# nilsbore/gp_compressor

Measured on AMD Instinct MI355X. Metric: patches/sec (compress+predict), higher is better.
Workload: dtype f64; 1 GPU; C2 room scan: 8192 patches x 256 pts per GPU, RBF + Gaussian noise, dense Cholesky fit + predictive mean on the 20x20 grid (m=400); patches_per_gpu=8192, points_per_patch=256, grid_points=400, parallelism=1 GPU, kernel=dense_mfma_w1

## Files before the change

### gp_compressor_amd/capi.py

```python
import ctypes as C
import os
import weakref

import numpy as np

HERE = os.path.dirname(os.path.abspath(__file__))
LIB_PATH = os.environ.get("GPC_LIB_PATH", os.path.join(HERE, "libgpc_hip.so"))

GPC_OK, GPC_EINVAL, GPC_ENOMEM, GPC_ENODEV, GPC_EHIP, GPC_ERANGE = 0, -22, -12, -19, -5, -34
CELL_UNOBSERVED, CELL_OCCUPIED, CELL_FREE = 0, 1, 2
STATUS_OK, STATUS_NOT_SPD, STATUS_NAN, STATUS_SIGMA_CLAMPED, STATUS_OVERFLOW, STATUS_NOT_CONVERGED = 0, 1, 2, 3, 4, 5
MAX_POINTS, MAX_BV = 1024, 256

c_dp = C.POINTER(C.c_double)
c_ip = C.POINTER(C.c_int32)


class Params(C.Structure):
    _fields_ = [("sigmaf_sq", C.c_double), ("l_sq", C.c_double), ("noise", C.c_double), ("eps_tol", C.c_double),
                ("capacity", C.c_int32), ("noise_model", C.c_int32), ("ref_double_noise", C.c_int32),
                ("ref_field_delete_bug", C.c_int32), ("want_variance", C.c_int32), ("reserved", C.c_int32)]


class IrlsParams(C.Structure):
# ... 143 lines not shown
    "gpc_registration_get_cloud": (C.c_int, [_vp, _vp]),
    "gpc_registration_cloud_dev": (C.c_int, [_vp, C.POINTER(_vp), C.POINTER(C.c_int)]),
    "gpc_registration_get_assignment": (C.c_int, [_vp, _vp, _vp]),
    "gpc_partition_patches": (C.c_int, [_i, _vp, _i, _i, _vp]),
    "gpc_comm_unique_id": (C.c_int, [_vp]),
    "gpc_comm_create": (C.c_int, [_vp, _i, _i, _vp, C.POINTER(_vp)]),
    "gpc_comm_create_all": (C.c_int, [_i, C.POINTER(_vp), C.POINTER(_vp)]),
    "gpc_comm_adopt": (C.c_int, [_vp, _vp, _i, _i, C.POINTER(_vp)]),
    "gpc_comm_destroy": (None, [_vp]),
    "gpc_comm_world": (C.c_int, [_vp]),
    "gpc_comm_rank": (C.c_int, [_vp]),
    "gpc_comm_library": (C.c_char_p, []),
    "gpc_comm_set_partition": (C.c_int, [_vp, _i, _vp]),
    "gpc_group_start": (C.c_int, []),
    "gpc_group_end": (C.c_int, []),
    "gpc_allgather_fstar_dev": (C.c_int, [_vp, _i, _vp, _vp, _vp]),
    "gpc_unpermute_fstar_dev": (C.c_int, [_vp, _i, _vp, _vp]),
    "gpc_test_exp_host": (None, [_vp, _vp, _i]),
    "gpc_test_exp_small_host": (None, [_vp, _vp, _i]),
    "gpc_test_quantize_host": (C.c_int, [_vp, _i, _i, _vp, _vp, _vp]),
    "gpc_test_rate_allocate_host": (C.c_int, [_i, _i, _vp, _vp, _vp, _vp, _d, _vp, _i, C.c_int64, _i, _vp, _vp, _vp, _vp]),
    "gpc_test_par_memcpy": (None, [_vp, _vp, C.c_size_t]),
    "gpc_test_dense_route": (C.c_int, [_i] * 11 + [_vp, _i, _vp]),
}

_lib = None


def load():
    global _lib
    if _lib is not None:
        return _lib
    try:
        import torch
    except ImportError:
        pass
    if not os.path.exists(LIB_PATH):
        raise GpcError(GPC_ENODEV, f"{LIB_PATH} not built: run `python -c 'import __graft_entry__ as g; g.build()'` "
                                   "(hipcc --offload-arch=gfx950); there is no CPU fallback")
    lib = C.CDLL(LIB_PATH)
    for name, (res, args) in PROTOTYPES.items():
        fn = getattr(lib, name)
        fn.restype = res
        fn.argtypes = args
    _lib = lib
    return lib
# ... 129 lines not shown
    def free_host_array(self, a):
        p = getattr(self, "_pinned", {}).pop(a.ctypes.data, None)
        if p is not None:
            self._check(self.lib.gpc_host_free(self.h, p))

    def rate_allocate(self, kmax, d0, d, need, w=None, w_all=1.0, unit=None, unit_all=24, refine=True, count=None):
        a = _rate_args(kmax, d0, d, w, unit, count)
        R, ld = a[2].shape
        k = np.zeros(R, dtype=np.int32)
        tg = None if count is None else np.zeros(R, dtype=np.int32)
        res = np.zeros(1, dtype=RATE_RESULT_DTYPE)
        self._check(self.lib.gpc_rate_allocate(self.h, R, ld, _ptr(a[0]), _ptr(a[1]), _ptr(a[2]), _ptr(a[3]), float(w_all), _ptr(a[4]),
                                               int(unit_all), int(need), int(bool(refine)), _ptr(a[5]), _ptr(k), _ptr(tg), _ptr(res)))
        return (k, rate_result(res)) if count is None else (k, tg, rate_result(res))

    def rate_allocate_dev(self, R, ld, kmax, d0, d, need, w=None, w_all=1.0, unit=None, unit_all=24, refine=True, count=None, k=None,
                          target=None, result=None):
        self._check(self.lib.gpc_rate_allocate_dev(self.h, int(R), int(ld), _ptr(kmax), _ptr(d0), _ptr(d), _ptr(w), float(w_all),
                                                   _ptr(unit), int(unit_all), int(need), int(bool(refine)), _ptr(count), _ptr(k),
                                                   _ptr(target), _ptr(result)))

    def last_dense_kernel(self):
        return self.lib.gpc_last_dense_kernel(self.h).decode()

    def dense_fit_predict(self, params, off, x0, x1, y, xs0, xs1, want_alpha=False):
        off = np.ascontiguousarray(off, dtype=np.int32)
        y = np.ascontiguousarray(np.atleast_2d(y), dtype=np.float64)
        x0 = np.ascontiguousarray(x0, dtype=np.float64)
        x1 = np.ascontiguousarray(x1, dtype=np.float64)
        xs0 = np.ascontiguousarray(xs0, dtype=np.float64)
        xs1 = np.ascontiguousarray(xs1, dtype=np.float64)
        P, ny, m = off.shape[0] - 1, y.shape[0], xs0.shape[0]
        f = np.full((P, ny, m), np.nan)
        v = np.full((P, m), np.nan) if params.want_variance else None
        st = np.full(P, -1, dtype=np.int32)
        al = np.full_like(y, np.nan) if want_alpha else None
        self._check(self.lib.gpc_dense_fit_predict(self.h, C.byref(params), P, _ptr(off), _ptr(x0), _ptr(x1), _ptr(y), ny,
                                                   m, _ptr(xs0), _ptr(xs1), _ptr(f), _ptr(v), _ptr(al), _ptr(st)))
        return (f, v, st, al) if want_alpha else (f, v, st)

    def dense_fit_predict_grid(self, params, off, x0, x1, y, res, sz, want_alpha=False):
        off = np.ascontiguousarray(off, dtype=np.int32)
        y = np.ascontiguousarray(np.atleast_2d(y), dtype=np.float64)
        x0 = np.ascontiguousarray(x0, dtype=np.float64)
        x1 = np.ascontiguousarray(x1, dtype=np.float64)
        P, ny, m = off.shape[0] - 1, y.shape[0], sz * sz
# ... 1080 lines not shown
    tg = None if count is None else np.zeros(R, dtype=np.int32)
    res = np.zeros(1, dtype=RATE_RESULT_DTYPE)
    rc = load().gpc_test_rate_allocate_host(R, ld, _ptr(a[0]), _ptr(a[1]), _ptr(a[2]), _ptr(a[3]), float(w_all), _ptr(a[4]), int(unit_all),
                                            int(need), int(bool(refine)), _ptr(a[5]), _ptr(k), _ptr(tg), _ptr(res))
    if rc != GPC_OK:
        raise GpcError(rc, "gpc_test_rate_allocate_host")
    return (k, rate_result(res)) if count is None else (k, tg, rate_result(res))


test_rate_allocate_host.__test__ = False


ROUTE_KINDS = {-1: "no route", 0: "nothing", 1: "one-wave", 2: "register", 3: "tiled", 4: "generic", 5: "split"}
ROUTE_SHAPE = ("w1_npad", "w1_slots", "nt", "export_factor", "waves", "npad", "per_cu", "nt17", "need_big")


def dense_route(P, n_max, n_total=None, ny=1, m=16, variance=False, pointwise=False, alpha_out=False, num_cus=256, irls=False,
                w1_refused=False):
    name = C.create_string_buffer(96)
    shape = np.zeros(len(ROUTE_SHAPE), dtype=np.int32)
    kind = load().gpc_test_dense_route(P, n_max, P * n_max if n_total is None else n_total, ny, m, int(variance), int(pointwise),
                                       int(alpha_out), num_cus, int(irls), int(w1_refused), name, len(name), _ptr(shape))
    return ROUTE_KINDS[kind], name.value.decode(), dict(zip(ROUTE_SHAPE, shape.tolist()))
```

### gp_compressor_amd/csrc/dense_api.hip

```cpp
#include "dense_internal.h"

int dense_check(gpc_ctx* ctx, const gpc_params* prm, int P, const void* off, int n_max, int n_total,
                const void* x0, const void* x1, const void* y, int ny, int m, const void* f_star)
{
    if (!ctx || ctx->dead.load()) return GPC_EINVAL;
    if (!prm) return gpc_fail(ctx, GPC_EINVAL, "params is NULL");
    if (P < 0 || m < 0 || n_total < 0 || n_max < 0) return gpc_fail(ctx, GPC_EINVAL, "negative size");
    if (ny != 1 && ny != 3) return gpc_fail(ctx, GPC_EINVAL, "ny must be 1 (depth) or 3 (RGB), got %d", ny);
    if (P > 0 && !off) return gpc_fail(ctx, GPC_EINVAL, "off is NULL");
    if (n_total > 0 && (!x0 || !x1 || !y)) return gpc_fail(ctx, GPC_EINVAL, "x0/x1/y is NULL");
    if (P > 0 && m > 0 && !f_star) return gpc_fail(ctx, GPC_EINVAL, "f_star is NULL");
    if (n_max > GPC_MAX_POINTS) return gpc_fail(ctx, GPC_ERANGE, "n_max %d > GPC_MAX_POINTS %d", n_max, GPC_MAX_POINTS);
    if (!(prm->l_sq > 0.0) || !(prm->sigmaf_sq >= 0.0) || !(prm->noise >= 0.0))
        return gpc_fail(ctx, GPC_EINVAL, "kernel/noise parameters out of range");
    return GPC_OK;
}

DenseArgs dense_args(const gpc_params* prm, int P, const int32_t* off, int n_max, int n_total, const double* x0, const double* x1,
                     const double* y, int ny, int m, double* f_star, double* alpha_out, int32_t* status)
{
    DenseArgs a{};
    a.prm = *prm;
    a.P = P; a.n_max = n_max; a.n_total = n_total; a.ny = ny; a.m = m;
    a.off = off; a.x0 = x0; a.x1 = x1; a.y = y;
// ... 75 lines not shown
    if (nt17 && (rc = run_class(1, c1, on_in)) != GPC_OK) return bail(rc);
    if ((rc = run_class(0, c0, site)) != GPC_OK) return bail(rc);
    GPC_HIP(ctx, hipEventRecord(ctx->ev[1][GPC_EV_CLASS_FORK], ctx->s_in));
    GPC_HIP(ctx, hipEventRecord(ctx->ev[2][GPC_EV_CLASS_FORK], ctx->s_out));
    GPC_HIP(ctx, hipStreamWaitEvent(main_s, ctx->ev[1][GPC_EV_CLASS_FORK], 0));
    GPC_HIP(ctx, hipStreamWaitEvent(main_s, ctx->ev[2][GPC_EV_CLASS_FORK], 0));
    return rc;
}

int dense_dispatch(gpc_ctx* ctx, DenseArgs& a, const DenseSite& site, unsigned* seen_gen)
{
    const DenseSwitches sw = dense_switches_read();
    const DenseFacts facts = dense_facts(ctx, a);
    DenseRoute route = dense_route(facts, sw);
    if (route.kind == DENSE_NOTHING) return GPC_OK;
    if (a.n_max < 1) a.n_max = 1;
    if (seen_gen)
        if (int rco = gpc_pipe_chunk_order(ctx, site.stream, seen_gen)) return rco;
    GPC_HIP(ctx, hipSetDevice(ctx->device));
    if (!a.prm.want_variance) a.v_star = nullptr;
    if (int rcp = gpc_debug_poison_lds(ctx, site)) return rcp;
    int grid = 0, rc = GPC_OK;
    if (route.kind == DENSE_ONE_WAVE) {
        for (int cap_w1 = site.w1_cap;;) {
            rc = gpc_ws_reserve(ctx, site, al256(dense_w1_ws_bytes(facts, route, &grid, cap_w1)));
            if (rc != GPC_ENOMEM) break;
            cap_w1 = grid / 2;
            if (cap_w1 < 4 * ctx->num_cus) break;
        }
        if (rc == GPC_ENOMEM) {
            route = dense_route(facts, sw, true);
            if (route.kind == DENSE_NO_ROUTE) return rc;
            (void)hipGetLastError();
        } else if (rc != GPC_OK) {
            return rc;
        }
    }
    switch (route.kind) {
        case DENSE_ONE_WAVE:
            rc = dense_w1_launch(ctx, site, a, route, grid);
            break;
        case DENSE_REGISTER:
            rc = dense_mfma_launch(ctx, site, a, route);
            break;
        case DENSE_TILED:
            if ((rc = gpc_ws_reserve(ctx, site, al256(dense_big_ws_bytes(ctx, a, route, &grid)))) == GPC_OK)
                rc = dense_big_launch(ctx, site, a, route, grid);
            break;
        case DENSE_SPLIT:
// ... 65 lines not shown
    if (ctx && (sz < 0 || sz > 1024)) return gpc_fail(ctx, GPC_EINVAL, "sz out of range");
    int rc = dense_check(ctx, params, P, off, n_max, n_total, x0, x1, y, ny, sz * sz, f_star);
    if (rc != GPC_OK) return rc;
    DenseArgs a = dense_args(params, P, off, n_max, n_total, x0, x1, y, ny, sz * sz, f_star, alpha_out, status);
    a.prm.want_variance = 0;
    a.grid_res = res; a.grid_sz = sz;
    std::lock_guard<std::mutex> lk(ctx->mu);
    return dense_dispatch(ctx, a, dense_site_of(ctx));
}

int gpc_test_dense_route(int P, int n_max, int n_total, int ny, int m, int variance, int pointwise, int alpha_out, int num_cus, int irls,
                         int w1_refused, char* name, int name_cap, int32_t* shape)
{
    const DenseFacts f{P, n_max, n_total, ny, m, variance != 0, pointwise != 0, alpha_out != 0, num_cus, irls != 0};
    const DenseRoute r = dense_route(f, dense_switches_read(), w1_refused != 0);
    if (name && name_cap > 0) snprintf(name, (size_t)name_cap, "%s", r.name);
    if (shape) {
        const int32_t v[GPC_TEST_ROUTE_SHAPE] = {r.w1_npad, r.w1_slots, r.nt, r.export_factor, r.waves, r.npad, r.per_cu, r.nt17, r.need_big};
        memcpy(shape, v, sizeof(v));
    }
    return (int)r.kind;
}

}
```

### gp_compressor_amd/csrc/dense_host.hip

```cpp
#include <algorithm>
#include <condition_variable>
#include <cstdlib>
#include <thread>
#include <vector>

#include "dense_internal.h"

namespace {
class CopyPool {
public:
    static CopyPool& get()
    {
        static CopyPool p;
        return p;
    }
    void copy(void* dst, const void* src, size_t bytes)
    {
        if (bytes < (1u << 20) || th_.empty()) { std::memcpy(dst, src, bytes); return; }
        std::lock_guard<std::mutex> call(call_mu_);
        std::unique_lock<std::mutex> lk(m_);
        dst_ = (char*)dst; src_ = (const char*)src; bytes_ = bytes;
        remaining_ = (int)th_.size();
        ++gen_;
        lk.unlock();
// ... 103 lines not shown
    struct PipeFlag {
        gpc_ctx* c;
        bool on;
        ~PipeFlag()
        {
            if (!on) return;
            std::lock_guard<std::mutex> lk(c->mu);
            c->pipe_active = false;
        }
    } pipe{ctx, false};
    {
        std::lock_guard<std::mutex> lk(ctx->mu);
        DenseFacts chunk{(P + 7) / 8, n_max, n_total, ny, m, want_v, !grid && xs0, false, ctx->num_cus, false};
        bool all_w1 = C == 4 && P >= 8192 && n_max > 160 && !alpha_out && !sw.host_one_stream && ctx->own_stream != nullptr;
        for (int c = 0; c < 8 && all_w1; ++c) {
            const int p0 = (int)((long long)P * c / 8), p1 = (int)((long long)P * (c + 1) / 8);
            DenseFacts fc = chunk;
            fc.P = p1 - p0;
            fc.n_max = 1;
            for (int i = p0; i < p1; ++i) fc.n_max = std::max(fc.n_max, off[i + 1] - off[i]);
            all_w1 = dense_route(fc, sw).kind == DENSE_ONE_WAVE;
        }
        if (all_w1) {
            half = (dense_w1_ws_bytes(chunk, dense_route(chunk, sw), nullptr) + 255) & ~(size_t)255;
            if (gpc_ws_reserve(ctx, 2 * half) == GPC_OK) {
                two = true;
                C = 8;
                pipe.on = ctx->pipe_active = true;
                seen_gen[0] = seen_gen[1] = ctx->foreign_gen;
            } else {
                (void)hipGetLastError();
            }
        }
    }
    auto al256 = [](size_t v) { return (v + 255) & ~(size_t)255; };
    const size_t b_off = al256(sizeof(int32_t) * (size_t)(P + C)), b_x = al256(8 * N), b_y = al256(8 * N * ny), b_xs = al256(8 * (size_t)m),
                 b_f = al256(8 * (size_t)P * ny * m), b_v = want_v ? al256(8 * (size_t)P * m) : 0, b_al = alpha_out ? al256(8 * N * ny) : 0,
                 b_st = al256(sizeof(int32_t) * (size_t)P);
    if ((rc = grow(ctx, &ctx->io, &ctx->io_bytes, b_off + 2 * b_x + b_y + 2 * b_xs + b_f + b_v + b_al + b_st, false))) return rc;
    char* d = static_cast<char*>(ctx->io);
    int32_t* d_off = (int32_t*)d; d += b_off;
    double* d_x0 = (double*)d; d += b_x;
    double* d_x1 = (double*)d; d += b_x;
    double* d_y = (double*)d; d += b_y;
    double* d_xs0 = (double*)d; d += b_xs;
    double* d_xs1 = (double*)d; d += b_xs;
    double* d_f = (double*)d; d += b_f;
// ... 137 lines not shown
```

### gp_compressor_amd/csrc/dense_internal.h

```cpp
#pragma once

#include "gpc_internal.h"
#include "dense_route.h"

struct DenseArgs {
    gpc_params prm;
    int P, n_max, n_total, ny, m;
    const int32_t* off;
    const double *x0, *x1, *y;
    const double *xs0, *xs1;
    double grid_res;
    int grid_sz;
    double *f_star, *v_star, *alpha_out;
    int32_t* status;
    const int32_t* sel;
    const int32_t* sel_count;
    int sel_base;
    double* log_ev;
};

struct DenseSite {
    hipStream_t stream;
    size_t ws_off, ws_len;
    int w1_cap = 0;
// ... 62 lines not shown
struct GaussRows {
    double *f;
    double *v;
    double *alpha;
    double *log_ev;
    int32_t *status;
};
int dense_gauss_keep_launch(gpc_ctx* ctx, const DenseSite& site, int h, int P, int ny, int m, int n_total, const int32_t* off,
                            const GaussRows& cand, const GaussRows& out, int32_t* best, double* log_ev_all_h, int32_t* cur_best,
                            double* cur_ev);
struct SelectRows {
    double *f, *v, *p;
    double *alpha, *fhat;
    double* log_q;
    int32_t *iters, *status;
};
int dense_select_keep_launch(gpc_ctx* ctx, const DenseSite& site, int h, int P, int m, const int32_t* off, const SelectRows& cand,
                             const SelectRows& out, int32_t* best, double* log_q_all_h, int32_t* cur_best, double* cur_lq);

size_t dense_big_ws_bytes(const gpc_ctx* ctx, const DenseArgs& a, const DenseRoute& r, int* grid_out);
int dense_big_launch(gpc_ctx* ctx, const DenseSite& site, const DenseArgs& a, const DenseRoute& r, int grid);
size_t dense_w1_ws_bytes(const DenseFacts& f, const DenseRoute& r, int* grid_out, int cap = 0);
int dense_w1_launch(gpc_ctx* ctx, const DenseSite& site, const DenseArgs& a, const DenseRoute& r, int grid);
struct IrlsArgs {
    int max_iter;
    double tol, f_init;
    int32_t* iters;
    double* fhat;
    double* s_out;
};
int dense_irls_launch(gpc_ctx* ctx, const DenseSite& site, const DenseArgs& a, const DenseRoute& r, const IrlsArgs& ir, int grid);
```

### gp_compressor_amd/csrc/dense_mfma_w1.hip

```cpp
#include <cstdio>
#include <cstdlib>
#include <type_traits>

#include "gpc_device.h"
#include "dense_internal.h"
#include "mfma_tile.h"

#define W1_NPAD_MAX 512
#define W1_C 4
#define W1_NDT 10
#define W1_NT_OF(npad) ((npad) / 16)
#define W1_TRI_OF(npad) (W1_NT_OF(npad) * (W1_NT_OF(npad) + 1) / 2)
#define W1_TILE(i, j) (((size_t)(i) * (size_t)((i) + 1) / 2 + (size_t)(j)) * MF_IMG)
#define W1_PACK_OF(npad) ((npad) <= 256)
#define W1_LNV_OF(npad) (W1_PACK_OF(npad) ? W1_NT_OF(npad) / 2 : W1_NT_OF(npad))


struct W1Params {
    DenseArgs a;
    double c_exp;
    double pivot_tol;
    double cs, noise_u, sfp, a_out;
    double* ws;
    double* linvt;
    int export_factor;
    unsigned long long* stamps;
};
#define W1_NPH 12
#ifdef W1_STAMPS
#define W1_STAMP(ph)                                                                                                 \
    do {                                                                                                             \
        __builtin_amdgcn_sched_barrier(0);                                                                           \
        const unsigned long long t_now_ = __builtin_amdgcn_s_memtime();                                              \
        st_acc_[ph] += t_now_ - t_prev_;                                                                             \
        t_prev_ = t_now_;                                                                                            \
        __builtin_amdgcn_sched_barrier(0);                                                                           \
    } while (0)
#else
#define W1_STAMP(ph) do { } while (0)
#endif

#define W1_LDS_SYNC()                                                                                                \
    do {                                                                                                             \
        __builtin_amdgcn_fence(__ATOMIC_SEQ_CST, "wavefront");                                                       \
        __builtin_amdgcn_wave_barrier();                                                                             \
    } while (0)

template <int A, int B, typename F>
// ... 55 lines not shown
#pragma unroll
            for (int q = 0; q < 4; ++q) v[t][q] *= sf;
    }
    if constexpr (DIAG) {
#pragma unroll
        for (int q = 0; q < 4; ++q) {
            double d = v[CNT - 1][q] + noise;
            if (dbl) d += noise;
            v[CNT - 1][q] = (lr == lg + 4 * q) ? d : v[CNT - 1][q];
        }
    }
    if (MF_TS * (r + 1) > n || MF_TS * (c0 + CNT) > n) {
#pragma unroll
        for (int t = 0; t < CNT; ++t) {
#pragma unroll
            for (int q = 0; q < 4; ++q) {
                const int pj = MF_TS * (c0 + t) + lg + 4 * q;
                if (pi >= n || pj >= n) v[t][q] = (pi == pj) ? 1.0 : 0.0;
            }
        }
    }
}

template <int W1_NPAD>
__global__ __launch_bounds__(64, 2) void dense_w1_kernel(W1Params g)
{
    constexpr int W1_NT = W1_NT_OF(W1_NPAD), W1_TRI = W1_TRI_OF(W1_NPAD);
    __shared__ __attribute__((aligned(16))) double T[GPC_EXP_TABLE_SIZE];
    __shared__ __attribute__((aligned(16))) double px0[W1_NPAD], px1[W1_NPAD], zv[W1_NPAD];
    __shared__ __attribute__((aligned(16))) double rsbuf[32], wsc[32];
    __shared__ __attribute__((aligned(16))) double LinvC[W1_C * MF_IMG];
    constexpr bool W1_PACK = W1_PACK_OF(W1_NPAD);
    constexpr int W1_LNV = W1_LNV_OF(W1_NPAD);
    __shared__ __attribute__((aligned(16))) double dgl[W1_PACK ? W1_LNV * MF_TS : 2];

    const DenseArgs& A = g.a;
    int lane = threadIdx.x;
    int lr = lane & 15, lg = lane >> 4;
#define W1_FRESH_LANE()                                                                                              \
    do {                                                                                                             \
        lane = mf_opaque(lane);                                                                                      \
        lr = lane & 15;                                                                                              \
        lg = lane >> 4;                                                                                              \
    } while (0)
    const int m = A.m;
    const double sf = A.prm.sigmaf_sq, cexp = g.c_exp;
    const bool dbl = A.prm.ref_double_noise != 0;
    const int patch = blockIdx.x;
    double* Lt = g.ws + (size_t)patch * W1_TRI * MF_IMG;
    double* LinvTg = g.linvt + (size_t)patch * W1_LNV * MF_IMG;

    gpc_exp_table_init(T);
    {
        const int o = __builtin_amdgcn_readfirstlane(A.off[patch]);
        const int n = __builtin_amdgcn_readfirstlane(A.off[patch + 1]) - o;
        double* fs = A.f_star + (size_t)patch * m;
        __syncthreads();
        if (n <= 0 || n > W1_NPAD) {
            for (int p = lane; p < m; p += 64) fs[p] = (n == 0) ? 0.0 : __builtin_nan("");
            if (lane == 0 && A.status) A.status[patch] = (n == 0) ? GPC_STATUS_OK : GPC_STATUS_NAN;
            return;
        }
        const int nt = __builtin_amdgcn_readfirstlane((n + MF_TS - 1) / MF_TS);
#ifdef W1_STAMPS
        unsigned long long st_acc_[W1_NPH] = {};
        unsigned long long t_prev_ = __builtin_amdgcn_s_memtime();
#endif

        const double xo0 = A.x0[o], xo1 = A.x1[o];
        double qr0[W1_NPAD / 64], qr1[W1_NPAD / 64];
        double mn0 = xo0, mx0 = xo0, mn1 = xo1, mx1 = xo1;
#pragma unroll
        for (int u = 0; u < W1_NPAD / 64; ++u) {
            const int i = lane + 64 * u;
            const bool live = i < n;
            qr0[u] = live ? A.x0[o + i] : xo0;
            qr1[u] = live ? A.x1[o + i] : xo1;
            mn0 = __builtin_fmin(mn0, qr0[u]); mx0 = __builtin_fmax(mx0, qr0[u]);
            mn1 = __builtin_fmin(mn1, qr1[u]); mx1 = __builtin_fmax(mx1, qr1[u]);
            zv[i] = live ? A.y[o + i] : 0.0;
        }
// ... 504 lines not shown
                    q1 = A.grid_res * (((double)gy + 0.5) / (double)A.grid_sz - 0.5);
                }
                q0 = cs * (q0 - co0);
                q1 = cs * (q1 - co1);
                double s_ = 0.0;
                for (int i = 0; i < n; ++i) {
                    const double d0 = px0[i] - q0, d1 = px1[i] - q1;
                    s_ += gpc_exp_neg(argc * __builtin_fma(d0, d0, d1 * d1), T) * av[i];
                }
                fs[p] = sfp * s_;
            }
        }
        if (lane == 0 && A.status) A.status[patch] = GPC_STATUS_OK;
#ifdef W1_STAMPS
        W1_STAMP(10);
        if (g.stamps && lane == 0)
            for (int q_ = 0; q_ < W1_NPH; ++q_) atomicAdd(g.stamps + q_, st_acc_[q_]);
#endif
    }
}

static_assert(W1_NPAD_MAX == 512, "dense_route (dense_route.h) names the instances: 256 and 512 points");

size_t dense_w1_ws_bytes(const DenseFacts& f, const DenseRoute& r, int* grid_out, int cap_in)
{
    const int cap = cap_in > 0 && cap_in < r.w1_slots ? cap_in : r.w1_slots;
    const int grid = f.P < cap ? f.P : cap;
    if (grid_out) *grid_out = grid;
    const int npad = r.w1_npad;
    return sizeof(double) * ((size_t)(W1_TRI_OF(npad) + W1_LNV_OF(npad)) * MF_IMG * (size_t)grid + (f.variance ? (size_t)f.n_total : 0));
}

int dense_w1_launch(gpc_ctx* ctx, const DenseSite& site, const DenseArgs& a_in, const DenseRoute& r, int grid)
{
    DenseArgs a = a_in;
    double* v_star = a.v_star;
    double* log_ev = a.log_ev;
    a.v_star = nullptr;
    a.log_ev = nullptr;
    const bool exported = v_star || log_ev;
    W1Params g;
    g.c_exp = (double)(-0.5f) / a.prm.l_sq;
    g.ws = reinterpret_cast<double*>(dense_ws(ctx, site));
    const int npad = r.w1_npad;
    g.linvt = g.ws + (size_t)W1_TRI_OF(npad) * MF_IMG * (size_t)grid;
    g.export_factor = exported ? 1 : 0;
    const double sf = a.prm.sigmaf_sq;
    const bool unit = !exported;
    g.cs = sqrt(-g.c_exp);
    g.noise_u = unit ? a.prm.noise / sf : a.prm.noise;
    g.pivot_tol = GPC_PIVOT_RTOL * (unit ? 1.0 + a.prm.noise / sf : sf + a.prm.noise);
    g.sfp = unit ? 1.0 : sf;
    g.a_out = unit ? 1.0 / sf : 1.0;
    g.stamps = nullptr;
    if (exported) {
        if (v_star) a.m = 0;
        if (!a.alpha_out) a.alpha_out = g.linvt + (size_t)W1_LNV_OF(npad) * MF_IMG * (size_t)grid;
    }
#ifdef W1_STAMPS
    if (getenv("GPC_W1_STAMPS")) {
        GPC_HIP(ctx, hipMalloc(&g.stamps, sizeof(unsigned long long) * W1_NPH));
        GPC_HIP(ctx, hipMemsetAsync(g.stamps, 0, sizeof(unsigned long long) * W1_NPH, site.stream));
    }
#endif
    for (int base = 0; base < a.P; base += grid) {
        const int cnt = a.P - base < grid ? a.P - base : grid;
        g.a = a;
        g.a.P = cnt;
        g.a.off = a.off + base;
        g.a.f_star = a.f_star ? a.f_star + (size_t)base * a.ny * a_in.m : nullptr;
        g.a.status = a.status ? a.status + base : nullptr;
        if (npad == 256) hipLaunchKernelGGL((dense_w1_kernel<256>), dim3(cnt), dim3(64), 0, site.stream, g);
        else hipLaunchKernelGGL((dense_w1_kernel<W1_NPAD_MAX>), dim3(cnt), dim3(64), 0, site.stream, g);
        GPC_HIP(ctx, hipGetLastError());
        if (v_star) {
            DenseArgs av = g.a;
            av.m = a_in.m;
            const int rc = dense_variance_launch(ctx, site, av, W1_NT_OF(256), r.var_w4, g.ws, a.alpha_out, v_star + (size_t)base * a_in.m);
            if (rc != GPC_OK) return rc;
        }
        if (log_ev) {
            const int rc = dense_gauss_evidence_launch(ctx, site, g.a, W1_NT_OF(256), 0, g.ws, 0, a.alpha_out, log_ev + (size_t)base * a.ny);
            if (rc != GPC_OK) return rc;
        }
    }
#ifdef W1_STAMPS
    if (g.stamps) {
        unsigned long long h[W1_NPH];
        GPC_HIP(ctx, hipStreamSynchronize(site.stream));
        GPC_HIP(ctx, hipMemcpy(h, g.stamps, sizeof(h), hipMemcpyDeviceToHost));
        (void)hipFree(g.stamps);
        static const char* names[W1_NPH] = {"load", "sweep gram", "sweep loop", "chain", "forward", "pass gram", "pass loop", "pass trsm",
                                            "step fence", "backward", "predict", ""};
        unsigned long long tot = 0;
        for (int q = 0; q < W1_NPH; ++q) tot += h[q];
        fprintf(stderr, "[GPC_W1_STAMPS] mean s_memtime ticks per patch (total %.0f)\n", (double)tot / a.P);
// ... 6 lines not shown
```

### gp_compressor_amd/csrc/dense_route.h

```cpp
#pragma once

#include <cstdlib>

#include "../../include/gpc.h"

struct DenseSwitches {
    bool force_generic, force_big;
    bool no_w1, no_w1_512, w2;
    bool w1_min_p_set;
    int w1_min_p;
    int w1_slots;
    bool no_split, no_nt17, no_hint;
    bool big_no_w2, big_no_w4;
    int var_w4;
    bool host_no_pipeline, host_one_stream;
};

static inline DenseSwitches dense_switches_read()
{
    DenseSwitches s{};
    s.force_generic = getenv("GPC_FORCE_GENERIC") != nullptr;
    s.force_big = getenv("GPC_FORCE_BIG") != nullptr;
    s.no_w1 = getenv("GPC_NO_W1") != nullptr;
    s.no_w1_512 = getenv("GPC_NO_W1_512") != nullptr;
    s.w2 = getenv("GPC_W2") != nullptr;
    const char* mp = getenv("GPC_W1_MIN_P");
    s.w1_min_p_set = mp != nullptr;
    s.w1_min_p = mp ? atoi(mp) : 0;
    const char* sl = getenv("GPC_W1_SLOTS");
    s.w1_slots = sl && atoi(sl) > 0 ? atoi(sl) : 0;
    s.no_split = getenv("GPC_NO_SPLIT") != nullptr;
    s.no_nt17 = getenv("GPC_NO_NT17") != nullptr;
    s.no_hint = getenv("GPC_NO_HINT") != nullptr;
    s.big_no_w2 = getenv("GPC_BIG_NO_W2") != nullptr;
    s.big_no_w4 = getenv("GPC_BIG_NO_W4") != nullptr;
    const char* vw = getenv("GPC_VAR_W4");
    s.var_w4 = vw ? (atoi(vw) != 0 ? 1 : 0) : -1;
    s.host_no_pipeline = getenv("GPC_HOST_NO_PIPELINE") != nullptr;
    s.host_one_stream = getenv("GPC_HOST_ONE_STREAM") != nullptr;
    return s;
}

struct DenseFacts {
    int P, n_max, n_total, ny, m;
    bool variance;
    bool pointwise;
    bool alpha_out;
    int num_cus;
    bool irls;
};

enum DenseKind {
    DENSE_NO_ROUTE = -1,
    DENSE_NOTHING = 0,
    DENSE_ONE_WAVE,
    DENSE_REGISTER,
    DENSE_TILED,
    DENSE_GENERIC,
    DENSE_SPLIT
};

#define DENSE_W1_MAX_SLOTS 8192

struct DenseRoute {
    DenseKind kind;
    const char* name;
    int w1_npad, w1_slots;
    int nt;
    bool export_factor;
    int waves, npad, per_cu;
    bool nt17, need_big;
    int var_w4;
};

static inline DenseRoute dense_route_register(int n_max, bool variance, int var_w4)
{
    static const char* const names[2][5] = {
        {"dense_mfma_nt4", "dense_mfma_nt8", "dense_mfma_nt12", "dense_mfma_nt16", "dense_mfma_nt17"},
        {"dense_mfma_nt4 + dense_variance", "dense_mfma_nt8 + dense_variance", "dense_mfma_nt12 + dense_variance",
         "dense_mfma_nt16 + dense_variance", ""}};
    const int i = n_max <= 64 ? 0 : n_max <= 128 ? 1 : n_max <= 192 ? 2 : n_max <= 256 ? 3 : 4;
    DenseRoute r{};
    r.kind = DENSE_REGISTER;
    r.nt = i < 4 ? 4 * (i + 1) : 17;
    r.export_factor = variance;
    r.name = names[variance][i];
    r.var_w4 = var_w4;
    return r;
}

// ... 30 lines not shown
}

static inline DenseRoute dense_route(const DenseFacts& f_in, const DenseSwitches& s, bool w1_refused = false)
{
    DenseFacts f = f_in;
    DenseRoute none{};
    none.kind = DENSE_NOTHING;
    none.name = "";
    if (f.P == 0 || (!f.irls && f.m == 0 && !f.alpha_out)) return none;
    if (f.n_max < 1) f.n_max = 1;
    if (f.irls) return dense_route_tiled(f, s);
    const int n = f.n_max;
    const bool v = f.variance, depth = f.ny == 1, ny_ok = f.ny == 1 || f.ny == 3;
    if (!s.force_generic && !s.force_big && ny_ok) {
        const bool no_split = f.P == 1 || s.no_split;
        const int min_p = s.w1_min_p_set ? s.w1_min_p : 4 * f.num_cus;
        const bool w1_can = depth && (v ? n <= 256 && n > 192 && f.pointwise : n <= 512);
        if (w1_can && f.P >= min_p && f.P > 1 && !s.no_w1 && !(n > 256 && s.no_w1_512)) {
            if (!w1_refused) {
                DenseRoute r{};
                r.kind = DENSE_ONE_WAVE;
                r.w1_npad = n <= 256 ? 256 : 512;
                r.w1_slots = s.w1_slots ? s.w1_slots : DENSE_W1_MAX_SLOTS;
                r.var_w4 = s.var_w4;
                r.name = v ? "dense_mfma_w1 + dense_variance" : n <= 256 ? "dense_mfma_w1" : "dense_mfma_w1_512";
                return r;
            }
            if (v) { none.kind = DENSE_NO_ROUTE; return none; }
        }
        if (n > 192 && n <= 256 && depth && !v && f.P > 1 && s.w2) return dense_route_tiled(f, s);
        if (n <= 256 || (no_split && n <= 17 * 16 && depth && !v && !s.no_nt17)) return dense_route_register(n, v, s.var_w4);
        const bool uniform = (long long)f.P * n == (long long)f.n_total;
        if (!v && n <= GPC_MAX_POINTS && !no_split && !(uniform && n > 17 * 16)) {
            DenseRoute r = dense_route_tiled(f, s);
            r.kind = DENSE_SPLIT;
            r.nt17 = depth && !s.no_nt17;
            r.need_big = !(r.nt17 && n <= 17 * 16);
            r.name = !r.need_big ? "dense_mfma_nt16 + dense_mfma_nt17" : r.nt17 ? "dense_mfma_nt16 + dense_mfma_nt17 + dense_mfma_big"
                                                                                 : "dense_mfma_nt16 + dense_mfma_big";
            return r;
        }
    }
    const bool big_can = n > 256 && n <= 1024 && (!v || f.pointwise) && ny_ok;
    if ((big_can || (s.force_big && n <= 1024 && !v)) && !s.force_generic) return dense_route_tiled(f, s);
    DenseRoute r{};
    r.kind = DENSE_GENERIC;
// ... 4 lines not shown
```

### gp_compressor_amd/csrc/gpc_api.hip

```cpp
#include <algorithm>
#include <cstdlib>
#include <numeric>
#include <vector>

#include "gpc_device.h"
#include "dense_internal.h"

extern "C" {

int gpc_version(void) { return GPC_VERSION; }

void gpc_default_params_dense(gpc_params* p)
{
    if (!p) return;
    std::memset(p, 0, sizeof(*p));
    p->sigmaf_sq = 0.05 * 0.05;
    p->l_sq = 3.0 * 3.0;
    p->noise = 0.04 * 0.04;
    p->eps_tol = 0.0;
    p->capacity = 0;
    p->noise_model = 0;
    p->ref_double_noise = 1;
    p->ref_field_delete_bug = 1;
    p->want_variance = 0;
// ... 123 lines not shown
    if (bytes == 0) return GPC_OK;
    if (!dst || !src) return gpc_fail(ctx, GPC_EINVAL, "dst/src is NULL");
    const hipMemcpyKind k = kind == GPC_COPY_H2D ? hipMemcpyHostToDevice : kind == GPC_COPY_D2H ? hipMemcpyDeviceToHost
                          : kind == GPC_COPY_D2D ? hipMemcpyDeviceToDevice : hipMemcpyDefault;
    if (k == hipMemcpyDefault) return gpc_fail(ctx, GPC_EINVAL, "kind must be GPC_COPY_H2D, _D2H or _D2D");
    GPC_HIP(ctx, hipSetDevice(ctx->device));
    hipStream_t s = gpc_stream_of(ctx);
    GPC_HIP(ctx, hipMemcpyAsync(dst, src, bytes, k, s));
    GPC_HIP(ctx, hipStreamSynchronize(s));
    return GPC_OK;
}

void gpc_ctx_destroy(gpc_ctx* ctx)
{
    if (!ctx || ctx->dead.load()) return;
    {
        std::lock_guard<std::mutex> lk(ctx->mu);
        (void)hipSetDevice(ctx->device);
        (void)hipStreamSynchronize(ctx->stream);
        if (ctx->ws) (void)hipFree(ctx->ws);
        ctx->ws = nullptr;
        if (ctx->tickets) (void)hipFree(ctx->tickets);
        ctx->tickets = nullptr;
        ctx->ws_bytes = 0;
        if (ctx->s_in) {
            (void)hipStreamSynchronize(ctx->s_in);
            (void)hipStreamSynchronize(ctx->s_out);
            (void)hipStreamDestroy(ctx->s_in);
            (void)hipStreamDestroy(ctx->s_out);
            if (ctx->s_c2) { (void)hipStreamSynchronize(ctx->s_c2); (void)hipStreamDestroy(ctx->s_c2); ctx->s_c2 = nullptr; }
            for (auto& row : ctx->ev)
                for (auto& e : row) if (e) (void)hipEventDestroy(e);
            ctx->s_in = ctx->s_out = nullptr;
        }
        if (ctx->io) (void)hipFree(ctx->io);
        if (ctx->pin_in) (void)hipHostFree(ctx->pin_in);
        if (ctx->pin_out) (void)hipHostFree(ctx->pin_out);
        ctx->io = ctx->pin_in = ctx->pin_out = nullptr;
        ctx->io_bytes = ctx->pin_in_bytes = ctx->pin_out_bytes = 0;
        if (ctx->own_stream) (void)hipStreamDestroy(ctx->own_stream);
        ctx->own_stream = nullptr;
        ctx->stream = nullptr;
        snprintf(ctx->err, sizeof(ctx->err), "the context has been destroyed");
        ctx->dead.store(true);
    }
    gpc_ctx_unref(ctx);
// ... 135 lines not shown
```

### gp_compressor_amd/csrc/gpc_internal.h

```cpp
#pragma once

#include <hip/hip_runtime.h>

#include <cstdarg>
#include <cstdlib>
#include <cstdint>
#include <cstdio>
#include <cstring>
#include <atomic>
#include <mutex>
#include <string>
#include <utility>
#include <vector>

#include "../../include/gpc.h"

#define GPC_PIVOT_RTOL 1e-14

struct gpc_ctx {
    int device = 0;
    hipStream_t own_stream = nullptr;
    hipStream_t stream = nullptr;
    int num_cus = 256;
    void* ws = nullptr;
    size_t ws_bytes = 0;
    int32_t* tickets = nullptr;
    void* io = nullptr;
    size_t io_bytes = 0;
    void* pin_in = nullptr;
    size_t pin_in_bytes = 0;
    void* pin_out = nullptr;
    size_t pin_out_bytes = 0;
    hipStream_t s_in = nullptr, s_out = nullptr, s_c2 = nullptr;
    bool pipe_active = false;
    unsigned foreign_gen = 0;
    hipEvent_t ev[3][16] = {};
    std::mutex host_mu;
    const int32_t* hint_off = nullptr;
    int hint_P = 0, hint_le256 = 0, hint_le272 = 0;
    std::mutex mu;
    char err[512] = {0};
    const char* last_dense_kernel = "";
    std::atomic<int> refs{1};
    std::atomic<bool> dead{false};
    std::vector<std::pair<const void*, uint64_t>> children;
    uint64_t next_serial = 1;
};

// ... 192 lines not shown
```

### include/gpc.h

```cpp
#ifndef GPC_H
#define GPC_H

#include <stddef.h>
#include <stdint.h>

#ifdef __cplusplus
extern "C" {
#endif

#define GPC_VERSION 100

#define GPC_OK 0
#define GPC_EINVAL (-22)
#define GPC_ENOMEM (-12)
#define GPC_ENODEV (-19)
#define GPC_EHIP (-5)
#define GPC_ERANGE (-34)

#define GPC_STATUS_OK 0
#define GPC_STATUS_NOT_SPD 1
#define GPC_STATUS_NAN 2
#define GPC_STATUS_SIGMA_CLAMPED 3
#define GPC_STATUS_OVERFLOW 4
#define GPC_STATUS_NOT_CONVERGED 5
// ... 299 lines not shown
int gpc_comm_create(gpc_ctx* ctx, int world, int rank, const void* id128, gpc_comm** out);
int gpc_comm_create_all(int ndev, gpc_ctx* const* ctxs, gpc_comm** out );
int gpc_comm_adopt(gpc_ctx* ctx, void* nccl_comm, int world, int rank, gpc_comm** out);
void gpc_comm_destroy(gpc_comm* c);
int gpc_comm_world(const gpc_comm* c);
int gpc_comm_rank(const gpc_comm* c);
const char* gpc_comm_library(void);
int gpc_comm_set_partition(gpc_comm* c, int P, const int32_t* slot_patch);
int gpc_group_start(void);
int gpc_group_end(void);
int gpc_allgather_fstar_dev(gpc_comm* c, int row_doubles, const double* local_f, double* gathered, double* f_star);
int gpc_unpermute_fstar_dev(gpc_comm* c, int row_doubles, const double* gathered, double* f_star);

void gpc_test_exp_host(const double* x, double* out, int n);
void gpc_test_exp_small_host(const double* x, double* out, int n);
int gpc_test_quantize_host(const double* v, int b, int w, uint16_t* q, float* range, double* deq);
int gpc_test_rate_allocate_host(int R, int ld, const int32_t* kmax, const double* d0, const double* d, const double* w, double w_all,
                                const int32_t* unit, int unit_all, int64_t need, int refine, const int32_t* count, int32_t* k, int32_t* target,
                                gpc_rate_result* result);
void gpc_test_par_memcpy(void* dst, const void* src, size_t bytes);
#define GPC_TEST_ROUTE_SHAPE 9
int gpc_test_dense_route(int P, int n_max, int n_total, int ny, int m, int variance, int pointwise, int alpha_out, int num_cus,
                         int irls, int w1_refused, char* name, int name_cap, int32_t* shape);

#ifdef __cplusplus
}
#endif
#endif
```

Measured before the change: 5.575 million patches/s.

## Index one-wave workspace by hardware residency slot instead of patch

The one-wave dense kernel now picks its Cholesky/L-inverse scratch slot from the hardware wave location (XCC, CU, SIMD, wave id read via s_getreg), mapped through a CU table built once by a probe kernel. Scratch then scales with resident waves rather than with the patch count, which shrinks the workspace, lets the kernel launch all patches at once, and aims to keep scratch hot in cache. The cost is a one-time probe launch, reliance on undocumented HW_ID register layouts, and a fallback that writes NaN for any wave whose place is not in the table.

```diff
diff --git a/gp_compressor_amd/capi.py b/gp_compressor_amd/capi.py
--- a/gp_compressor_amd/capi.py
+++ b/gp_compressor_amd/capi.py
@@ -189,6 +189,9 @@
     "gpc_test_rate_allocate_host": (C.c_int, [_i, _i, _vp, _vp, _vp, _vp, _d, _vp, _i, C.c_int64, _i, _vp, _vp, _vp, _vp]),
     "gpc_test_par_memcpy": (None, [_vp, _vp, C.c_size_t]),
     "gpc_test_dense_route": (C.c_int, [_i] * 11 + [_vp, _i, _vp]),
+    "gpc_test_w1_slot_index": (C.c_int, [_i, _i, _i, _i, _vp]),
+    "gpc_test_w1_place": (None, [C.c_uint, C.c_uint, _vp]),
+    "gpc_debug_w1_places": (C.c_int, [_vp]),
 }
 
 _lib = None
@@ -364,6 +367,9 @@
 
     def last_dense_kernel(self):
         return self.lib.gpc_last_dense_kernel(self.h).decode()
+
+    def w1_places(self):
+        return self.lib.gpc_debug_w1_places(self.h)
 
     def dense_fit_predict(self, params, off, x0, x1, y, xs0, xs1, want_alpha=False):
         off = np.ascontiguousarray(off, dtype=np.int32)
@@ -1490,3 +1496,15 @@
     kind = load().gpc_test_dense_route(P, n_max, P * n_max if n_total is None else n_total, ny, m, int(variance), int(pointwise),
                                        int(alpha_out), num_cus, int(irls), int(w1_refused), name, len(name), _ptr(shape))
     return ROUTE_KINDS[kind], name.value.decode(), dict(zip(ROUTE_SHAPE, shape.tolist()))
+
+
+def w1_slot_index(cu, simd, wave, num_cus=256):
+    count = C.c_int(0)
+    slot = load().gpc_test_w1_slot_index(int(cu), int(simd), int(wave), int(num_cus), C.byref(count))
+    return slot, count.value
+
+
+def w1_place(hw_id, xcc_id):
+    fields = np.zeros(3, dtype=np.int32)
+    load().gpc_test_w1_place(int(hw_id), int(xcc_id), _ptr(fields))
+    return tuple(fields.tolist())
diff --git a/gp_compressor_amd/csrc/dense_api.hip b/gp_compressor_amd/csrc/dense_api.hip
--- a/gp_compressor_amd/csrc/dense_api.hip
+++ b/gp_compressor_amd/csrc/dense_api.hip
@@ -121,9 +121,10 @@
     if (int rcp = gpc_debug_poison_lds(ctx, site)) return rcp;
     int grid = 0, rc = GPC_OK;
     if (route.kind == DENSE_ONE_WAVE) {
+        if ((rc = dense_w1_settle(ctx, site, route)) != GPC_OK) return rc;
         for (int cap_w1 = site.w1_cap;;) {
             rc = gpc_ws_reserve(ctx, site, al256(dense_w1_ws_bytes(facts, route, &grid, cap_w1)));
-            if (rc != GPC_ENOMEM) break;
+            if (rc != GPC_ENOMEM || route.w1_residency) break;
             cap_w1 = grid / 2;
             if (cap_w1 < 4 * ctx->num_cus) break;
         }
@@ -235,4 +236,23 @@
     return (int)r.kind;
 }
 
-}
+int gpc_debug_w1_places(gpc_ctx* ctx)
+{
+    if (!ctx || ctx->dead.load()) return GPC_EINVAL;
+    std::lock_guard<std::mutex> lk(ctx->mu);
+    return ctx->w1_cus;
+}
+
+int gpc_test_w1_slot_index(int cu, int simd, int wave, int num_cus, int* count)
+{
+    if (count) *count = w1_slot_count(num_cus);
+    return w1_slot_index(cu, simd, wave, num_cus);
+}
+void gpc_test_w1_place(unsigned hw_id, unsigned xcc_id, int32_t* fields)
+{
+    fields[0] = w1_cu_key(hw_id, xcc_id);
+    fields[1] = w1_hw_simd(hw_id);
+    fields[2] = w1_hw_wave(hw_id);
+}
+
+}
diff --git a/gp_compressor_amd/csrc/dense_host.hip b/gp_compressor_amd/csrc/dense_host.hip
--- a/gp_compressor_amd/csrc/dense_host.hip
+++ b/gp_compressor_amd/csrc/dense_host.hip
@@ -149,7 +149,9 @@
             all_w1 = dense_route(fc, sw).kind == DENSE_ONE_WAVE;
         }
         if (all_w1) {
-            half = (dense_w1_ws_bytes(chunk, dense_route(chunk, sw), nullptr) + 255) & ~(size_t)255;
+            DenseRoute chunk_route = dense_route(chunk, sw);
+            if ((rc = dense_w1_settle(ctx, dense_site_of(ctx), chunk_route)) != GPC_OK) return rc;
+            half = (dense_w1_ws_bytes(chunk, chunk_route, nullptr) + 255) & ~(size_t)255;
             if (gpc_ws_reserve(ctx, 2 * half) == GPC_OK) {
                 two = true;
                 C = 8;
diff --git a/gp_compressor_amd/csrc/dense_internal.h b/gp_compressor_amd/csrc/dense_internal.h
--- a/gp_compressor_amd/csrc/dense_internal.h
+++ b/gp_compressor_amd/csrc/dense_internal.h
@@ -108,6 +108,7 @@
 int dense_big_launch(gpc_ctx* ctx, const DenseSite& site, const DenseArgs& a, const DenseRoute& r, int grid);
 size_t dense_w1_ws_bytes(const DenseFacts& f, const DenseRoute& r, int* grid_out, int cap = 0);
 int dense_w1_launch(gpc_ctx* ctx, const DenseSite& site, const DenseArgs& a, const DenseRoute& r, int grid);
+int dense_w1_settle(gpc_ctx* ctx, const DenseSite& site, DenseRoute& r);
 struct IrlsArgs {
     int max_iter;
     double tol, f_init;
diff --git a/gp_compressor_amd/csrc/dense_mfma_w1.hip b/gp_compressor_amd/csrc/dense_mfma_w1.hip
--- a/gp_compressor_amd/csrc/dense_mfma_w1.hip
+++ b/gp_compressor_amd/csrc/dense_mfma_w1.hip
@@ -24,6 +24,8 @@
     double* ws;
     double* linvt;
     int export_factor;
+    const int32_t* cu_map;
+    int num_cus;
     unsigned long long* stamps;
 };
 #define W1_NPH 12
@@ -125,7 +127,7 @@
     }
 }
 
-template <int W1_NPAD>
+template <int W1_NPAD, bool RES>
 __global__ __launch_bounds__(64, 2) void dense_w1_kernel(W1Params g)
 {
     constexpr int W1_NT = W1_NT_OF(W1_NPAD), W1_TRI = W1_TRI_OF(W1_NPAD);
@@ -150,8 +152,18 @@
     const double sf = A.prm.sigmaf_sq, cexp = g.c_exp;
     const bool dbl = A.prm.ref_double_noise != 0;
     const int patch = blockIdx.x;
-    double* Lt = g.ws + (size_t)patch * W1_TRI * MF_IMG;
-    double* LinvTg = g.linvt + (size_t)patch * W1_LNV * MF_IMG;
+    size_t slot_at = (size_t)patch;
+    bool no_place = false;
+    if constexpr (RES) {
+        const unsigned hw = __builtin_amdgcn_s_getreg(4 | (0 << 6) | (15 << 11));
+        const unsigned xcc = __builtin_amdgcn_s_getreg(20 | (0 << 6) | (3 << 11));
+        const int cu = __builtin_amdgcn_readfirstlane(g.cu_map[w1_cu_key(hw, xcc)]);
+        const int slot = w1_slot_index(cu, w1_hw_simd(hw), w1_hw_wave(hw), g.num_cus);
+        no_place = slot < 0;
+        slot_at = (size_t)((unsigned)__builtin_amdgcn_readfirstlane(no_place ? 0 : slot) & W1_SLOT_MASK);
+    }
+    double* Lt = g.ws + slot_at * W1_TRI * MF_IMG;
+    double* LinvTg = g.linvt + slot_at * W1_LNV * MF_IMG;
 
     gpc_exp_table_init(T);
     {
@@ -159,7 +171,7 @@
         const int n = __builtin_amdgcn_readfirstlane(A.off[patch + 1]) - o;
         double* fs = A.f_star + (size_t)patch * m;
         __syncthreads();
-        if (n <= 0 || n > W1_NPAD) {
+        if (n <= 0 || n > W1_NPAD || (RES && no_place)) {
             for (int p = lane; p < m; p += 64) fs[p] = (n == 0) ? 0.0 : __builtin_nan("");
             if (lane == 0 && A.status) A.status[patch] = (n == 0) ? GPC_STATUS_OK : GPC_STATUS_NAN;
             return;
@@ -710,13 +722,59 @@
 
 static_assert(W1_NPAD_MAX == 512, "dense_route (dense_route.h) names the instances: 256 and 512 points");
 
+static int w1_slots_of(const DenseFacts& f, const DenseRoute& r, int grid) { return r.w1_residency ? w1_slot_count(f.num_cus) : grid; }
+
 size_t dense_w1_ws_bytes(const DenseFacts& f, const DenseRoute& r, int* grid_out, int cap_in)
 {
     const int cap = cap_in > 0 && cap_in < r.w1_slots ? cap_in : r.w1_slots;
-    const int grid = f.P < cap ? f.P : cap;
+    const int grid = r.w1_residency || f.P < cap ? f.P : cap;
     if (grid_out) *grid_out = grid;
     const int npad = r.w1_npad;
-    return sizeof(double) * ((size_t)(W1_TRI_OF(npad) + W1_LNV_OF(npad)) * MF_IMG * (size_t)grid + (f.variance ? (size_t)f.n_total : 0));
+    return sizeof(double) * ((size_t)(W1_TRI_OF(npad) + W1_LNV_OF(npad)) * MF_IMG * (size_t)w1_slots_of(f, r, grid) +
+                             (f.variance ? (size_t)f.n_total : 0));
+}
+
+__global__ __launch_bounds__(64) void dense_w1_probe_kernel(int32_t* keys)
+{
+    extern __shared__ double w1_probe_lds[];
+    const unsigned hw = __builtin_amdgcn_s_getreg(4 | (0 << 6) | (15 << 11));
+    const unsigned xcc = __builtin_amdgcn_s_getreg(20 | (0 << 6) | (3 << 11));
+    const int key = w1_cu_key(hw, xcc);
+    w1_probe_lds[threadIdx.x] = (double)key;
+    __syncthreads();
+    for (int k = 0; k < 8; ++k) __builtin_amdgcn_s_sleep(127);
+    if (threadIdx.x == 0) keys[blockIdx.x] = (int32_t)w1_probe_lds[0];
+}
+
+int dense_w1_settle(gpc_ctx* ctx, const DenseSite& site, DenseRoute& r)
+{
+    if (r.kind != DENSE_ONE_WAVE || !r.w1_residency) return GPC_OK;
+    if (ctx->w1_cus == 0) {
+        const int grid = ctx->num_cus * 4, lds = 160 * 1024;
+        std::vector<int32_t> keys((size_t)grid), map(W1_CU_KEYS, -1);
+        int32_t* d_keys = nullptr;
+        GPC_HIP(ctx, hipFuncSetAttribute(reinterpret_cast<const void*>(dense_w1_probe_kernel), hipFuncAttributeMaxDynamicSharedMemorySize, lds));
+        GPC_HIP(ctx, hipMalloc(&d_keys, sizeof(int32_t) * (size_t)grid));
+        hipLaunchKernelGGL(dense_w1_probe_kernel, dim3(grid), dim3(64), lds, site.stream, d_keys);
+        hipError_t e = hipGetLastError();
+        if (e == hipSuccess) e = hipMemcpyAsync(keys.data(), d_keys, sizeof(int32_t) * (size_t)grid, hipMemcpyDeviceToHost, site.stream);
+        if (e == hipSuccess) e = hipStreamSynchronize(site.stream);
+        (void)hipFree(d_keys);
+        GPC_HIP(ctx, e);
+        int found = 0;
+        for (int32_t k : keys)
+            if (k >= 0 && k < W1_CU_KEYS) map[(size_t)k] = 0;
+        for (int32_t& v : map)
+            if (v == 0) v = found++;
+        ctx->w1_cus = -1;
+        if (found == ctx->num_cus && (unsigned)w1_slot_count(found) <= W1_SLOT_MASK + 1u) {
+            GPC_HIP(ctx, hipMalloc(&ctx->w1_cu_map, sizeof(int32_t) * W1_CU_KEYS));
+            GPC_HIP(ctx, hipMemcpy(ctx->w1_cu_map, map.data(), sizeof(int32_t) * W1_CU_KEYS, hipMemcpyHostToDevice));
+            ctx->w1_cus = found;
+        }
+    }
+    if (ctx->w1_cus != ctx->num_cus) r.w1_residency = false;
+    return GPC_OK;
 }
 
 int dense_w1_launch(gpc_ctx* ctx, const DenseSite& site, const DenseArgs& a_in, const DenseRoute& r, int grid)
@@ -731,8 +789,13 @@
     g.c_exp = (double)(-0.5f) / a.prm.l_sq;
     g.ws = reinterpret_cast<double*>(dense_ws(ctx, site));
     const int npad = r.w1_npad;
-    g.linvt = g.ws + (size_t)W1_TRI_OF(npad) * MF_IMG * (size_t)grid;
+    const bool residency = r.w1_residency && !exported && r.w1_npad == 256 && ctx->w1_cu_map && ctx->w1_cus == ctx->num_cus;
+    if (r.w1_residency && !residency) return gpc_fail(ctx, GPC_EINVAL, "one-wave kernel: residency slots without the table of places, or with the export");
+    const int slots = residency ? w1_slot_count(ctx->num_cus) : grid;
+    g.linvt = g.ws + (size_t)W1_TRI_OF(npad) * MF_IMG * (size_t)slots;
     g.export_factor = exported ? 1 : 0;
+    g.cu_map = residency ? ctx->w1_cu_map : nullptr;
+    g.num_cus = ctx->num_cus;
     const double sf = a.prm.sigmaf_sq;
     const bool unit = !exported;
     g.cs = sqrt(-g.c_exp);
@@ -743,7 +806,7 @@
     g.stamps = nullptr;
     if (exported) {
         if (v_star) a.m = 0;
-        if (!a.alpha_out) a.alpha_out = g.linvt + (size_t)W1_LNV_OF(npad) * MF_IMG * (size_t)grid;
+        if (!a.alpha_out) a.alpha_out = g.linvt + (size_t)W1_LNV_OF(npad) * MF_IMG * (size_t)slots;
     }
 #ifdef W1_STAMPS
     if (getenv("GPC_W1_STAMPS")) {
@@ -758,8 +821,9 @@
         g.a.off = a.off + base;
         g.a.f_star = a.f_star ? a.f_star + (size_t)base * a.ny * a_in.m : nullptr;
         g.a.status = a.status ? a.status + base : nullptr;
-        if (npad == 256) hipLaunchKernelGGL((dense_w1_kernel<256>), dim3(cnt), dim3(64), 0, site.stream, g);
-        else hipLaunchKernelGGL((dense_w1_kernel<W1_NPAD_MAX>), dim3(cnt), dim3(64), 0, site.stream, g);
+        if (residency) hipLaunchKernelGGL((dense_w1_kernel<256, true>), dim3(cnt), dim3(64), 0, site.stream, g);
+        else if (npad == 256) hipLaunchKernelGGL((dense_w1_kernel<256, false>), dim3(cnt), dim3(64), 0, site.stream, g);
+        else hipLaunchKernelGGL((dense_w1_kernel<W1_NPAD_MAX, false>), dim3(cnt), dim3(64), 0, site.stream, g);
         GPC_HIP(ctx, hipGetLastError());
         if (v_star) {
             DenseArgs av = g.a;
diff --git a/gp_compressor_amd/csrc/dense_route.h b/gp_compressor_amd/csrc/dense_route.h
--- a/gp_compressor_amd/csrc/dense_route.h
+++ b/gp_compressor_amd/csrc/dense_route.h
@@ -3,6 +3,7 @@
 #include <cstdlib>
 
 #include "../../include/gpc.h"
+#include "dense_w1_slot.h"
 
 struct DenseSwitches {
     bool force_generic, force_big;
@@ -10,6 +11,7 @@
     bool w1_min_p_set;
     int w1_min_p;
     int w1_slots;
+    int w1_slot_per_patch;
     bool no_split, no_nt17, no_hint;
     bool big_no_w2, big_no_w4;
     int var_w4;
@@ -29,6 +31,8 @@
     s.w1_min_p = mp ? atoi(mp) : 0;
     const char* sl = getenv("GPC_W1_SLOTS");
     s.w1_slots = sl && atoi(sl) > 0 ? atoi(sl) : 0;
+    const char* spp = getenv("GPC_W1_SLOT_PER_PATCH");
+    s.w1_slot_per_patch = spp ? (atoi(spp) != 0 ? 1 : 0) : -1;
     s.no_split = getenv("GPC_NO_SPLIT") != nullptr;
     s.no_nt17 = getenv("GPC_NO_NT17") != nullptr;
     s.no_hint = getenv("GPC_NO_HINT") != nullptr;
@@ -66,6 +70,7 @@
     DenseKind kind;
     const char* name;
     int w1_npad, w1_slots;
+    bool w1_residency;
     int nt;
     bool export_factor;
     int waves, npad, per_cu;
@@ -142,6 +147,8 @@
                 r.kind = DENSE_ONE_WAVE;
                 r.w1_npad = n <= 256 ? 256 : 512;
                 r.w1_slots = s.w1_slots ? s.w1_slots : DENSE_W1_MAX_SLOTS;
+                r.w1_residency = !v && !s.w1_slots && n <= 256 &&
+                                 (s.w1_slot_per_patch < 0 ? f.P >= w1_slot_count(f.num_cus) : s.w1_slot_per_patch == 0);
                 r.var_w4 = s.var_w4;
                 r.name = v ? "dense_mfma_w1 + dense_variance" : n <= 256 ? "dense_mfma_w1" : "dense_mfma_w1_512";
                 return r;
diff --git a/gp_compressor_amd/csrc/dense_w1_slot.h b/gp_compressor_amd/csrc/dense_w1_slot.h
--- /dev/null
+++ b/gp_compressor_amd/csrc/dense_w1_slot.h
@@ -0,0 +1,25 @@
+#pragma once
+
+#if defined(__HIPCC__)
+#define W1_SLOT_HD __host__ __device__
+#else
+#define W1_SLOT_HD
+#endif
+
+#define W1_WAVE_SLOTS 8
+#define W1_SIMDS 4
+#define W1_CU_KEYS 4096
+
+W1_SLOT_HD constexpr int w1_cu_key(unsigned hw_id, unsigned xcc_id) { return (int)(((xcc_id & 15u) << 8) | ((hw_id >> 8) & 255u)); }
+W1_SLOT_HD constexpr int w1_hw_simd(unsigned hw_id) { return (int)((hw_id >> 4) & 3u); }
+W1_SLOT_HD constexpr int w1_hw_wave(unsigned hw_id) { return (int)(hw_id & 15u); }
+
+#define W1_SLOT_MASK 0xffffu
+
+W1_SLOT_HD constexpr int w1_slot_count(int num_cus) { return num_cus > 0 ? num_cus * W1_SIMDS * W1_WAVE_SLOTS : 0; }
+W1_SLOT_HD constexpr int w1_slot_index(int cu, int simd, int wave, int num_cus)
+{
+    return (cu < 0 || cu >= num_cus || simd < 0 || simd >= W1_SIMDS || wave < 0 || wave >= W1_WAVE_SLOTS)
+               ? -1
+               : (cu * W1_SIMDS + simd) * W1_WAVE_SLOTS + wave;
+}
diff --git a/gp_compressor_amd/csrc/gpc_api.hip b/gp_compressor_amd/csrc/gpc_api.hip
--- a/gp_compressor_amd/csrc/gpc_api.hip
+++ b/gp_compressor_amd/csrc/gpc_api.hip
@@ -169,6 +169,9 @@
         ctx->ws = nullptr;
         if (ctx->tickets) (void)hipFree(ctx->tickets);
         ctx->tickets = nullptr;
+        if (ctx->w1_cu_map) (void)hipFree(ctx->w1_cu_map);
+        ctx->w1_cu_map = nullptr;
+        ctx->w1_cus = 0;
         ctx->ws_bytes = 0;
         if (ctx->s_in) {
             (void)hipStreamSynchronize(ctx->s_in);
diff --git a/gp_compressor_amd/csrc/gpc_internal.h b/gp_compressor_amd/csrc/gpc_internal.h
--- a/gp_compressor_amd/csrc/gpc_internal.h
+++ b/gp_compressor_amd/csrc/gpc_internal.h
@@ -24,6 +24,8 @@
     int num_cus = 256;
     void* ws = nullptr;
     size_t ws_bytes = 0;
+    int32_t* w1_cu_map = nullptr;
+    int w1_cus = 0;
     int32_t* tickets = nullptr;
     void* io = nullptr;
     size_t io_bytes = 0;
diff --git a/include/gpc.h b/include/gpc.h
--- a/include/gpc.h
+++ b/include/gpc.h
@@ -345,6 +345,9 @@
 #define GPC_TEST_ROUTE_SHAPE 9
 int gpc_test_dense_route(int P, int n_max, int n_total, int ny, int m, int variance, int pointwise, int alpha_out, int num_cus,
                          int irls, int w1_refused, char* name, int name_cap, int32_t* shape);
+int gpc_test_w1_slot_index(int cu, int simd, int wave, int num_cus, int* count);
+int gpc_debug_w1_places(gpc_ctx* ctx);
+void gpc_test_w1_place(unsigned hw_id, unsigned xcc_id, int32_t* fields);
 
 #ifdef __cplusplus
 }
```

After: 5.545 million patches/s. Within noise of the previous version (-0.5%).
